# wizardyesterday/RtlSdrDiags

Hardware: AMD Instinct MI355X
Metric: IQ MSamples/s through WBFM chain at 1/2/4/8 GPUs; % HBM roofline (higher is better)
Workload: dtype int8/int16 Q15 + f32; 1 GPU; BASELINE configs[1]: WBFM, 1 channel, 2^28-sample synthetic IQ; channels_per_gpu=1, log2_samples_per_channel=28, kernels=streaming pipelines

## Files before the change

rtlsdrdiags_amd/csrc/iqd_engine.cpp:

```cpp
#include "iqdemod.h"

#include <hip/hip_runtime.h>
#include <math.h>
#include <stdarg.h>
#include <stdio.h>
#include <string.h>

#include <algorithm>
#include <mutex>
#include <string>
#include <vector>

#include "iqd_host.h"
#include "iqd_plan.h"
#include "iqd_kernels.h"
#include "iqd_stream.h"
#include "iqd_stream_mixed.h"
#include "iqd_taps.h"
#include "iqd_wbfm.h"
#include "iqd_chains.h"
#include "iqd_chan.h"

using namespace iqd;

// ... 61 lines not shown
    uint32_t *d_tracker = nullptr;
    AgcConfig *d_agc_cfg = nullptr;
    AgcState *d_agc = nullptr;
    GainEpoch *d_epochs = nullptr;
    std::vector<float> k_applied;
    std::vector<uint32_t> wbfm_epoch_left;
    std::vector<uint32_t> wbfm_epoch_seq;
    uint32_t accept_seq = 0;
    uint32_t *h_epoch_report = nullptr;
    bool epoch_report_pending = false;
    uint32_t epoch_report_seq = 0;
    std::vector<uint32_t> epoch_report_channels;
    uint32_t wbfm_epochs_live = 0;
    std::vector<int32_t> rot_applied;
    bool rot_changed = false;
    ScanConfig *d_scan_cfg = nullptr;
    ScanState *d_scan = nullptr;
    float *d_atan = nullptr, *d_fmlut = nullptr;
    float *d_half_lut = nullptr;
    uint32_t *d_amat[3] = {nullptr, nullptr, nullptr};
    uint32_t *d_amat4 = nullptr;
    D4Args d4_args{};
    std::vector<float> fm_kmax;
    bool stream_ok = false;
    std::vector<uint32_t> mode_gen, rot_gen;
    std::vector<float> wbfm_kmax;
    StreamArgs stream_args{};
    uint64_t stream_handoffs = 0;
    uint32_t *d_counters = nullptr;
    unsigned long long *d_stamps = nullptr;
    uint32_t *h_counters = nullptr;

    DevBuf stream_hist;
    DevBuf lists[FAM_COUNT + 1], mag_sums, blk_lists, vlen, records, base8k, base8k2, gain_trace, freq_trace, dc_records, dc_records2, repair_flags;
    size_t mag_sums_zero = 0;
    hipStream_t pre_stream = nullptr;
    hipEvent_t ev_pre_done[2] = {nullptr, nullptr}, ev_chain_done[2] = {nullptr, nullptr}, ev_main_decisions = nullptr;
    DevBuf g_sums[2], g_blk[2], g_vlen[2];
    int gate_set = 0;
    bool chain_pending[2] = {false, false};
    bool decisions_on_main = false;
    bool in_host_path = false;
    DevBuf st_iq, st_pcm, st_count, st_mag, st_allowed;
    DevBuf sl_iq[2], sl_pcm[2], sl_count[2], sl_mag[2], sl_allowed[2];
    hipStream_t copy_stream = nullptr;
    hipStream_t fam_stream[3] = {};
    hipEvent_t fam_fork = nullptr, fam_join[3] = {};
    hipEvent_t ev_in[2] = {nullptr, nullptr}, ev_free[2] = {nullptr, nullptr};
    uint32_t *h_slice_counts = nullptr;
    uint32_t *d_closed = nullptr, *h_closed = nullptr;
    size_t h_slice_counts_cap = 0;
    uint8_t *h_small = nullptr;
    size_t h_small_cap = 0;

    bool profiling = false;
    std::vector<std::pair<hipEvent_t, hipEvent_t>> ev_free_pairs, ev_pending;
    iqd_stats stats{};
    std::string last_error;

    int fail(int code, const char *fmt, ...)
    {
        char buf[512];
        va_list ap;
        va_start(ap, fmt);
        vsnprintf(buf, sizeof(buf), fmt, ap);
        va_end(ap);
        last_error = buf;
// ... 229 lines not shown
        ok = ok && hipMemcpyAsync(e->d_atan, atan_lut.data(), atan_lut.size() * sizeof(float),
                                  hipMemcpyHostToDevice, e->stream) == hipSuccess;
        ok = ok && hipMemcpyAsync(e->d_fmlut, fm_lut.data(), fm_lut.size() * sizeof(float),
                                  hipMemcpyHostToDevice, e->stream) == hipSuccess;
        ok = ok && hipMemcpyAsync(e->d_half_lut, half_lut.data(), half_lut.size() * sizeof(float),
                                  hipMemcpyHostToDevice, e->stream) == hipSuccess;
        for (int r = 0; r < 3; r++)
            ok = ok && hipMemcpyAsync(e->d_amat[r], amat[r].data(), amat[r].size() * sizeof(uint32_t),
                                      hipMemcpyHostToDevice, e->stream) == hipSuccess;
        ok = ok && hipMemcpyAsync(e->d_amat4, amat4.data(), amat4.size() * sizeof(uint32_t), hipMemcpyHostToDevice,
                                  e->stream) == hipSuccess;
        ok = ok && upload_consts(e->consts, e->stream) == hipSuccess;
        ok = ok && hipStreamSynchronize(e->stream) == hipSuccess;
    }
    if (!ok) {
        iqd_destroy(e);
        return IQD_ENOMEM;
    }
    *out = e;
    return IQD_OK;
}

void iqd_destroy(iqd_t *e)
{
    if (!e) return;
    (void)hipSetDevice(e->device);
    if (e->stream) (void)hipStreamSynchronize(e->stream);
    void *ptrs[] = {e->d_params, e->d_tails, e->d_wcarry, e->d_dc, e->d_tracker, e->d_agc_cfg, e->d_agc, e->d_epochs, e->d_scan_cfg, e->d_scan,
                    e->d_atan, e->d_fmlut, e->d_counters, e->d_stamps, e->d_half_lut, e->d_amat[0], e->d_amat[1], e->d_amat[2], e->d_amat4};
    for (void *p : ptrs)
        if (p) (void)hipFree(p);
    if (e->h_counters) (void)hipHostFree(e->h_counters);
    for (auto &b : e->lists) b.release();
    DevBuf *bufs[] = {&e->stream_hist, &e->mag_sums, &e->blk_lists, &e->vlen, &e->records, &e->base8k, &e->base8k2, &e->gain_trace, &e->freq_trace, &e->dc_records, &e->dc_records2, &e->repair_flags,
                      &e->st_iq, &e->st_pcm, &e->st_count, &e->st_mag, &e->st_allowed};
    for (DevBuf *b : bufs) b->release();
    for (int b = 0; b < 2; b++) {
        e->sl_iq[b].release(); e->sl_pcm[b].release(); e->sl_count[b].release();
        e->sl_mag[b].release(); e->sl_allowed[b].release();
        if (e->ev_in[b]) (void)hipEventDestroy(e->ev_in[b]);
        if (e->ev_free[b]) (void)hipEventDestroy(e->ev_free[b]);
    }
    if (e->pre_stream) {
        (void)hipStreamSynchronize(e->pre_stream);
        (void)hipStreamDestroy(e->pre_stream);
        for (int k = 0; k < 2; k++) {
            (void)hipEventDestroy(e->ev_pre_done[k]);
            (void)hipEventDestroy(e->ev_chain_done[k]);
            e->g_sums[k].release(); e->g_blk[k].release(); e->g_vlen[k].release();
        }
        (void)hipEventDestroy(e->ev_main_decisions);
    }
    if (e->h_slice_counts) (void)hipHostFree(e->h_slice_counts);
    if (e->h_small) (void)hipHostFree(e->h_small);
    if (e->h_epoch_report) (void)hipHostFree(e->h_epoch_report);
    if (e->d_closed) (void)hipFree(e->d_closed);
    if (e->h_closed) (void)hipHostFree(e->h_closed);
    if (e->copy_stream) (void)hipStreamDestroy(e->copy_stream);
    for (int f = 0; f < 3; f++) {
        if (e->fam_stream[f]) (void)hipStreamDestroy(e->fam_stream[f]);
        if (e->fam_join[f]) (void)hipEventDestroy(e->fam_join[f]);
    }
    if (e->fam_fork) (void)hipEventDestroy(e->fam_fork);
    for (auto *v : {&e->ev_free_pairs, &e->ev_pending})
        for (auto &pr : *v) { (void)hipEventDestroy(pr.first); (void)hipEventDestroy(pr.second); }
    if (e->stream) (void)hipStreamDestroy(e->stream);
    delete e;
// ... 934 lines not shown
    }
    if (f == FAM_WBFM) {
        HIP_TRY(e, e->records.ensure((size_t)n_list * a.tiles_per_ch * sizeof(WbfmRecord)));
        a.records = e->records.as<WbfmRecord>();
        if (e->repair_flags.cap < n_list * sizeof(uint32_t)) {
            HIP_TRY(e, e->repair_flags.ensure(n_list * sizeof(uint32_t)));
            HIP_COPY(e, hipMemsetAsync(e->repair_flags.p, 0, e->repair_flags.cap, s));
        }
        a.repair_flags = e->repair_flags.as<uint32_t>();
        if (streams) {
            const int stream_rot = e->plan_shape.fam[FAM_WBFM].rot_first;
            StreamArgs sa = e->stream_args;
            sa.amat = e->d_amat[stream_rot + 1];
            sa.half_lut = e->d_half_lut;
            sa.n_segments = n_list * a.tiles_per_ch;
            sa.grouped = fp.grouped ? 1u : 0u;
            for (int r = 0; r < 3; r++) {
                sa.group_start[r] = fp.grouped ? fp.group_start[r] : 0u;
                sa.group_li0[r] = fp.grouped ? fp.group_li0[r] : 0u;
                sa.group_nseg[r] = fp.grouped ? fp.group_nseg[r] : 0u;
                sa.amat3[r] = e->d_amat[2 - r];
            }
            sa.group_start[3] = fp.grouped ? fp.group_start[3] : 0u;
            sa.rounds = fp.rounds;
            sa.rings = fp.rings;
            HIP_TRY(e, e->stream_hist.ensure((size_t)sa.n_segments * sizeof(StHist)));
            sa.hist = e->stream_hist.as<StHist>();
            a.verify_at_end = x.gated ? 2u : 1u;
            if (fused) {
                x.mix.a[f] = a;
                x.mix.sa = sa;
                x.mix.wbfm_rot = stream_rot;
            } else {
                HIP_LAUNCH(e, launch_wbfm_stream(a, sa, stream_rot, x.fused_mag, fp.epochs, fp.grid, s));
                HIP_LAUNCH(e, launch_wbfm_stream_fixup(a, sa, s));
            }
            if (!x.gated) e->stream_handoffs += (uint64_t)n_list * ((x.vlen + a.tile_len - 1) / a.tile_len - 1);
            e->stats.stream_launches++;
        } else {
            HIP_LAUNCH(e, launch_wbfm(a, x.gated, x.fused_mag, n_list * a.tiles_per_ch, s));
        }
    } else {
        D4Args d4 = e->d4_args;
        if (streams) {
            for (int r = 0; r < 3; r++) {
                d4.group_start[r] = fp.group_start[r];
                d4.group_li0[r] = fp.group_li0[r];
                d4.group_nseg[r] = fp.group_nseg[r];
            }
            d4.group_start[3] = fp.group_start[3];
            d4.amat = e->d_amat4 + (size_t)(f == FAM_FM ? 0 : 3) * 4 * 64 * 4;
            d4.fm_lut = e->d_fmlut;
            d4.halo = (int32_t)fp.halo;
            d4.lead_shift = fp.lead_shift;
            d4.rounds = fp.rounds;
            d4.rings = fp.rings;
        }
        if (f != FAM_FM) {
            int rc = attach_dc_buffers(e, x, f, a, s);
            if (rc != IQD_OK) return rc;
            if (streams) {
                a.base_stride_ch = x.base.pcm_stride;
                a.base_stride_t = 1;
                static const bool no_det16 = getenv("IQD_NO_DET16") != nullptr;
                a.det16 = a.dc_tiles < 2 && !no_det16 ? 1u : 0u;
            }
        }
        if (streams) {
// ... 431 lines not shown
```

rtlsdrdiags_amd/csrc/iqd_kernels.hip:

```cpp
#include <hip/hip_runtime.h>

#include "iqd_kernels.h"
#include "iqd_chains.h"
#include "iqd_wbfm.h"
#include "iqd_stream_fix.h"

namespace iqd {

__constant__ Consts g_consts;

hipError_t upload_consts(const Consts &c, hipStream_t s)
{
    return hipMemcpyToSymbolAsync(HIP_SYMBOL(g_consts), &c, sizeof(Consts), 0, hipMemcpyHostToDevice, s);
}

hipError_t consts_address(const Consts **p)
{
    void *a = nullptr;
    const hipError_t e = hipGetSymbolAddress(&a, HIP_SYMBOL(g_consts));
    *p = (const Consts *)a;
    return e;
}

struct DeviceExec {
// ... 477 lines not shown
{
    if (blockIdx.x < a.n_list) tail_update_body(a, family, blockIdx.x);
    else squelch_block_body(q, always_open, (blockIdx.x - a.n_list) * 256u + threadIdx.x);
}

__global__ __launch_bounds__(256) void tail_dc_squelch_kernel(const ChainLaunch a, int family, const SquelchLaunch q, int always_open)
{
    __shared__ DcLds lds;
    if (blockIdx.x < a.n_list) {
        if (threadIdx.x >= 64) return;
        dc_channel_wave(a, family, blockIdx.x, lds);
    } else if (blockIdx.x < 2 * a.n_list) {
        tail_update_body(a, family, blockIdx.x - a.n_list);
    } else {
        squelch_block_body(q, always_open, (blockIdx.x - 2 * a.n_list) * 256u + threadIdx.x);
    }
}

__global__ __launch_bounds__(WB_THREADS, IQD_WBFM_MIN_WAVES) void wbfm_repair_squelch_kernel(const ChainLaunch a, const SquelchLaunch q, int always_open)
{
    __shared__ WbfmLds lds;
    if (blockIdx.x < a.n_list) wbfm_repair_body<false>(a, lds, blockIdx.x);
    else squelch_block_body(q, always_open, (blockIdx.x - a.n_list) * 256u + threadIdx.x);
}

struct MixedTailRoles { uint32_t end[6]; };
__global__ __launch_bounds__(256) void mixed_tail_kernel(const ChainLaunch a_wbfm, const StreamArgs sa, const ChainLaunch a_am,
                                                         const ChainLaunch a_fm, const ChainLaunch a_ssb, const MixedTailRoles roles)
{
    __shared__ union Lds { DcLds dc; FixLds fix; __device__ Lds() {} } u;
    DcLds &lds = u.dc;
    const uint32_t b = blockIdx.x;
    if (b < roles.end[0]) {
        wbfm_stream_fixup_body(a_wbfm, sa, b, u.fix);
    } else if (b < roles.end[2]) {
        if (threadIdx.x >= 64) return;
        const int family = b < roles.end[1] ? FAM_AM : FAM_SSB;
        const ChainLaunch &a = family == FAM_AM ? a_am : a_ssb;
        const uint32_t li = b - (family == FAM_AM ? roles.end[0] : roles.end[1]);
        dc_channel_wave(a, family, li, lds);
    } else if (b < roles.end[3]) {
        tail_update_body(a_am, FAM_AM, b - roles.end[2]);
    } else if (b < roles.end[4]) {
        tail_update_body(a_fm, FAM_FM, b - roles.end[3]);
    } else if (b < roles.end[5]) {
        tail_update_body(a_ssb, FAM_SSB, b - roles.end[4]);
    }
}

__global__ void squelch_track_kernel(const SquelchLaunch q, int always_open)
{
    const uint32_t ch = blockIdx.x * blockDim.x + threadIdx.x;
    if (ch >= q.n_ch) return;
    const uint32_t ech = q.first_ch + ch;
    const AgcConfig cfg = q.agc_cfg[ech];
    if (always_open && !cfg.enabled) return;
    const ChanParams &p = q.params[ech];
    AgcState st = q.agc[ech];
    uint32_t gain = st.rx_gain;
    uint32_t tracking = q.tracker[ech];
    uint32_t open = 0;
    const ScanConfig sc = q.scan_cfg[ech];
    ScanState ss = q.scan[ech];
    for (uint32_t b = 0; b < q.n_blocks; b++) {
        const size_t idx = (size_t)ch * q.n_blocks + b;
        const uint32_t avg = q.mag_sums[idx] / q.block_samples;
        if (!always_open) {
// ... 534 lines not shown
```

rtlsdrdiags_amd/csrc/iqd_stream.h:

```cpp
#pragma once
#include <stdint.h>

#include "iqd_device.h"

namespace iqd {

constexpr int ST_WAVES = 15;
constexpr int ST_THREADS = 64 * ST_WAVES;
constexpr int ST_RINGS = 3;
constexpr int ST_P_PER_RING = 4;
constexpr int ST_SEGS = 64 * ST_RINGS;
constexpr int ST_HALO = FORCED_BACK;
#ifndef IQD_ST_AHEAD
#define IQD_ST_AHEAD 2
#endif
constexpr int ST_AHEAD = IQD_ST_AHEAD;
constexpr int ST_MIN_TILE = 768;
constexpr int ST_FIX_PCM = 21;
constexpr int ST_ROW_FLOATS = 260;
#ifndef IQD_ST_FAKE_SHIFT
#define IQD_ST_FAKE_SHIFT 0
#endif
constexpr int ST_LDS_ROW_FLOATS = IQD_ST_FAKE_SHIFT ? (256 >> IQD_ST_FAKE_SHIFT) + 4 : ST_ROW_FLOATS;
constexpr int ST_TABLE_BYTES = 129 * ST_LDS_ROW_FLOATS * 4;
constexpr int ST_SLOT_BYTES = 64 * 16 * 4;
#ifndef IQD_ST_DEPTH
#define IQD_ST_DEPTH 1
#endif
constexpr int ST_DEPTH = IQD_ST_DEPTH;
constexpr int ST_RING_SLOTS = 2 * ST_DEPTH;
constexpr int ST_SYNC_WORDS = 24;
constexpr int ST_LDS_BYTES = ST_TABLE_BYTES + ST_RINGS * ST_RING_SLOTS * ST_SLOT_BYTES + ST_SYNC_WORDS * 4;
static_assert(ST_LDS_BYTES <= 160 * 1024, "table + rings must fit the CU's LDS");
static_assert(ST_HALO % 128 == 0 && ST_HALO + 32 <= TAIL, "the lead-in is whole 128-sample units inside the kept tail");

struct StHist {
    uint32_t w_first[2];
    uint32_t y1_first[6];
    uint32_t y2_first[24];
    uint32_t y1_last[4];
    uint32_t w_last[2];
    uint32_t pad[6];
    uint32_t y2_last[20];
};
static_assert(sizeof(StHist) == 256, "one boundary record per segment, 256 bytes");

struct StreamArgs {
    StHist *hist;
    const uint32_t *amat;
    const float *half_lut;
    uint32_t n_segments;
    uint32_t rounds;
    uint32_t rings;
    uint32_t grouped;
    uint32_t group_start[4];
    uint32_t group_li0[3];
    uint32_t group_nseg[3];
    const uint32_t *amat3[3];
    uint32_t d1p[4];
    uint32_t d1p2[4];
    uint32_t p12p[6];
    uint32_t a40p[20];
    float b0, a1;
};

enum { D4_AM = 0, D4_SSB = 1, D4_FM = 2 };
constexpr int D4_HALO_AM = fir_halo(FAM_AM), D4_HALO_SSB = fir_halo(FAM_SSB), D4_HALO_FM = fir_halo(FAM_FM);
constexpr int D4_HALO_SHORT = 128;
constexpr int d4_full_halo(int family) { return family == FAM_FM ? D4_HALO_FM : family == FAM_AM ? D4_HALO_AM : D4_HALO_SSB; }
constexpr int d4_lead_shift(int family) { return d4_full_halo(family) - D4_HALO_SHORT; }
constexpr int D4_REPLAY_AM = 4, D4_REPLAY_SSB = 36, D4_REPLAY_FM = 20;
constexpr int D4_REPLAY_PAIRS_AMSSB = 4;
constexpr int D4_RAILS_FROM_PIECE = 8;
constexpr int d4_replay_outputs(int family) { return family == FAM_FM ? D4_REPLAY_FM : family == FAM_AM ? D4_REPLAY_AM : D4_REPLAY_SSB; }
struct D4Geom { int64_t v0; uint32_t skip, cold; };
#if defined(__HIPCC__)
__host__ __device__
#endif
inline D4Geom d4_geom(uint32_t sid, uint32_t tile, uint32_t tile_len, uint32_t shift)
{
    D4Geom g;
    if (!shift) { g.v0 = (int64_t)tile * tile_len; g.skip = 0; g.cold = 1; return g; }
    g.cold = tile == 0 || (sid & 63u) == 0 ? 1u : 0u;
    const uint32_t c = 1u + (sid >> 6) - ((sid - tile) >> 6);
    g.v0 = (int64_t)tile * tile_len - (int64_t)shift * c;
    g.skip = g.cold ? shift : 0u;
    return g;
}
constexpr uint32_t d4_max_cold(uint32_t n_tiles) { return 1u + (n_tiles + 62u) / 64u; }
struct D4Args {
    const uint32_t *amat;
    const float *fm_lut;
    uint32_t group_start[4];
    uint32_t group_li0[3];
    uint32_t group_nseg[3];
    uint32_t rounds;
// ... 16 lines not shown
```

rtlsdrdiags_amd/csrc/iqd_stream.hip:

```cpp
#include <hip/hip_runtime.h>

#include "iqd_kernels.h"
#include "iqd_stream.h"
#include "iqd_wbfm.h"
#include "iqd_mfma.h"
#include "iqd_stream_fix.h"
#include "iqd_taps.h"

namespace iqd {

#ifdef IQD_ST_WT_STORES
__device__ __forceinline__ void st_store16(void *p, v4u v)
{
    asm volatile("global_store_dwordx4 %0, %1, off sc1\n\ts_nop 1" :: "v"(p), "v"(v) : "memory");
}
#define ST_STORE16(P, A, B, C, D) st_store16((void *)(P), v4u{A, B, C, D})
#elif defined(IQD_ST_NT_STORES)
#define ST_STORE16(P, A, B, C, D) __builtin_nontemporal_store(v4u{A, B, C, D}, (v4u *)(P))
#else
#define ST_STORE16(P, A, B, C, D) (*(u32x4 *)(P) = u32x4{A, B, C, D})
#endif


typedef __attribute__((address_space(3))) const uint32_t lds_cu32;
// ... 670 lines not shown
__device__ __forceinline__ void wbfm_stream_body(const ChainLaunch &a, const StreamArgs &sa, uint8_t *st_lds)
{
    if ((uint32_t)(uintptr_t)(__attribute__((address_space(3))) uint8_t *)st_lds != 0u) __builtin_trap();
    uint32_t *sync = (uint32_t *)(st_lds + ST_TABLE_BYTES + ST_RINGS * ST_RING_SLOTS * ST_SLOT_BYTES);
    const int tid = (int)threadIdx.x;
    {
        constexpr int N16 = ST_TABLE_BYTES / 16, TRIPS = (N16 + ST_THREADS - 1) / ST_THREADS;
        uint4 t[TRIPS];
#pragma unroll
        for (int k = 0; k < TRIPS; k++) {
            const int i = tid + k * ST_THREADS;
            t[k] = ((const uint4 *)sa.half_lut)[i < N16 ? i : N16 - 1];
        }
#pragma unroll
        for (int k = 0; k < TRIPS; k++) {
            const int i = tid + k * ST_THREADS;
            if (i < N16) ((uint4 *)st_lds)[i] = t[k];
        }
    }
    if (tid < ST_SYNC_WORDS) sync[tid] = 0;
    __syncthreads();
    const int wave = __builtin_amdgcn_readfirstlane(tid >> 6), lane = tid & 63;
    uint32_t pc = 0;
    if (wave < ST_RINGS) st_iir_wave(a, sa, st_lds, sync, wave, lane, ROT != 2 && !GATED && !EPOCHS ? IQD_ST_COLD_HALO : ST_HALO);
    else if (ROT != 2) st_p_wave<ROT, MAG, EPOCHS, GATED>(a, sa, st_lds, sync, wave - ST_RINGS, lane, pc);
    else {
        st_p_wave<1, MAG, EPOCHS, GATED, true>(a, sa, st_lds, sync, wave - ST_RINGS, lane, pc);
        st_p_wave<0, MAG, EPOCHS, GATED, true>(a, sa, st_lds, sync, wave - ST_RINGS, lane, pc);
        st_p_wave<-1, MAG, EPOCHS, GATED, true>(a, sa, st_lds, sync, wave - ST_RINGS, lane, pc);
    }
}

#ifndef IQD_STREAM_BODIES_ONLY
template <int ROT, bool MAG, bool EPOCHS, bool GATED>
__global__ __launch_bounds__(ST_THREADS, 4) void wbfm_stream_kernel(const ChainLaunch a, const StreamArgs sa)
{
    extern __shared__ __attribute__((aligned(16))) uint8_t st_lds[];
    wbfm_stream_body<ROT, MAG, EPOCHS, GATED>(a, sa, st_lds);
}
#endif

#ifndef IQD_STREAM_BODIES_ONLY
__global__ __launch_bounds__(FIX_THREADS) void wbfm_stream_fixup_kernel(const ChainLaunch a, const StreamArgs sa)
{
    __shared__ FixLds fl;
    wbfm_stream_fixup_body(a, sa, blockIdx.x, fl);
}

hipError_t launch_wbfm_stream_fixup(const ChainLaunch &a, const StreamArgs &sa, hipStream_t s)
{
    hipLaunchKernelGGL(wbfm_stream_fixup_kernel, dim3((sa.n_segments + FIX_SEGS - 1) / FIX_SEGS), dim3(FIX_THREADS), 0, s, a, sa);
    return hipGetLastError();
}

typedef void (*StKernel)(const ChainLaunch, const StreamArgs);
#define ST_K(R) {{wbfm_stream_kernel<R, false, false, false>, wbfm_stream_kernel<R, false, true, false>}, \
                 {wbfm_stream_kernel<R, true, false, false>, wbfm_stream_kernel<R, true, true, false>},   \
                 {wbfm_stream_kernel<R, false, false, true>, wbfm_stream_kernel<R, false, true, true>}}
static const StKernel st_kernels[4][3][2] = {ST_K(-1), ST_K(0), ST_K(1), ST_K(2)};
#undef ST_K

hipError_t init_wbfm_stream_kernels()
{
    for (int r = 0; r < 4; r++)
        for (int g = 0; g < 6; g++) {
            const hipError_t e = hipFuncSetAttribute((const void *)st_kernels[r][g >> 1][g & 1], hipFuncAttributeMaxDynamicSharedMemorySize, ST_LDS_BYTES);
            if (e != hipSuccess) return e;
        }
    return hipSuccess;
}

hipError_t launch_wbfm_stream(const ChainLaunch &a, const StreamArgs &sa, int rotation, bool mag, bool epochs, uint32_t grid, hipStream_t s)
{
    const int variant = a.vlen_gated ? 2 : (mag ? 1 : 0);
    hipLaunchKernelGGL(st_kernels[sa.grouped ? 3 : rotation < 0 ? 0 : rotation > 0 ? 2 : 1][variant][epochs ? 1 : 0], dim3(grid), dim3(ST_THREADS), ST_LDS_BYTES, s, a, sa);
    return hipGetLastError();
}

#endif

}
```

rtlsdrdiags_amd/csrc/iqd_stream_fix.h:

```cpp
#pragma once
#include <hip/hip_runtime.h>

#include "iqd_kernels.h"
#include "iqd_stream.h"
#include "iqd_stream_mixed.h"
#include "iqd_wbfm.h"
#include "iqd_mfma.h"

namespace iqd {

struct StSeg {
    uint32_t valid, li, tile, ch, ech;
    int32_t v0, tlen;
    int32_t vlen;
};

__device__ __forceinline__ StSeg st_segment(const ChainLaunch &a, uint32_t sid, uint32_t n_segments)
{
    StSeg s;
    s.valid = sid < n_segments ? 1u : 0u;
    const uint32_t id = s.valid ? sid : 0u;
    s.li = id / a.tiles_per_ch;
    s.tile = id - s.li * a.tiles_per_ch;
    s.ch = a.ch_list[s.li];
    s.ech = a.first_ch + s.ch;
    const uint32_t vlen = a.vlen_gated ? a.vlen_gated[s.ch] : a.vlen;
    s.vlen = (int32_t)vlen;
    const int64_t v0 = (int64_t)s.tile * a.tile_len;
    if (v0 >= (int64_t)vlen) { s.valid = 0; s.v0 = 0; s.tlen = 0; return s; }
    s.v0 = (int32_t)v0;
    const int64_t rest = (int64_t)vlen - v0;
    s.tlen = (int32_t)(rest < (int64_t)a.tile_len ? rest : (int64_t)a.tile_len);
    if (!s.valid) s.tlen = 0;
    return s;
}

#ifndef IQD_ST_NO_GROUPS
#define IQD_ST_NO_GROUPS 0
#endif
__device__ __forceinline__ StSeg st_segment_of(const ChainLaunch &a, const StreamArgs &sa, uint32_t sid, int &rot)
{
    if (IQD_ST_NO_GROUPS || !sa.grouped) { rot = 0; return st_segment(a, sid, sa.n_segments); }
    const uint32_t r = (sid >= sa.group_start[1] ? 1u : 0u) + (sid >= sa.group_start[2] ? 1u : 0u);
    rot = 1 - (int)r;
    const uint32_t local = sid - sa.group_start[r];
    const bool there = sid < sa.group_start[3] && local < sa.group_nseg[r];
    return st_segment(a, there ? sa.group_li0[r] * a.tiles_per_ch + local : sa.n_segments, sa.n_segments);
}
__device__ __forceinline__ bool st_cold_and_full(const StSeg &s, uint32_t tile_len)
{
    if (!s.valid) return true;
    const bool not_last = s.vlen - s.v0 > s.tlen;
    const bool keeps_restart = not_last && s.vlen - FORCED_BACK >= s.v0 && s.vlen - FORCED_BACK < s.v0 + s.tlen;
    return s.tile != 0 && s.tlen == (int32_t)tile_len && !keeps_restart;
}
__device__ __forceinline__ uint32_t st_id_count(const StreamArgs &sa) { return !IQD_ST_NO_GROUPS && sa.grouped ? sa.group_start[3] : sa.n_segments; }

#ifndef IQD_FIX_LANES
#define IQD_FIX_LANES 16
#endif
constexpr int FIX_LANES = IQD_FIX_LANES;
constexpr int FIX_SEGS = 256 / FIX_LANES;
constexpr int FIX_THREADS = FIX_LANES * FIX_SEGS;
static_assert(FIX_LANES == 16 || FIX_LANES == 32, "threads per boundary");
struct FixLds {
    uint32_t rec[(FIX_SEGS + 1) * 64];
    uint32_t y2x[FIX_SEGS][41];
};
__device__ __forceinline__ void wbfm_stream_fixup_body(const ChainLaunch &a, const StreamArgs &sa, const uint32_t block, FixLds &fl)
{
    uint32_t (&rec)[(FIX_SEGS + 1) * 64] = fl.rec;
    uint32_t (&y2x)[FIX_SEGS][41] = fl.y2x;
    const uint32_t sid0 = block * FIX_SEGS;
    const int tid = (int)threadIdx.x, sl = tid / FIX_LANES, i = tid % FIX_LANES;
    const uint32_t sid = sid0 + (uint32_t)sl;
    const StSeg sg = st_segment(a, sid < sa.n_segments ? sid : 0u, sa.n_segments);
    const bool live = sid < sa.n_segments && sg.valid && sg.tile != 0;
    float y_in = 0.f, y_end = 0.f;
    if (live && i == FIX_LANES - 1) {
        const WbfmRecord *r = a.records + (size_t)sg.li * a.tiles_per_ch;
        y_in = r[sg.tile].y_in;
        y_end = r[sg.tile - 1].y_end;
    }
    {
        const uint32_t *src = (const uint32_t *)sa.hist + ((size_t)sid0 - (sid0 ? 1 : 0)) * 64;
        const uint32_t n_avail = (sa.n_segments - sid0 < (uint32_t)FIX_SEGS ? sa.n_segments - sid0 : (uint32_t)FIX_SEGS) + (sid0 ? 1u : 0u);
        for (uint32_t k = (uint32_t)tid; k < n_avail * 64; k += FIX_THREADS) rec[k + (sid0 ? 0 : 64)] = src[k];
    }
    __syncthreads();
    const StHist &prev = *(const StHist *)&rec[sl * 64], &own = *(const StHist *)&rec[(sl + 1) * 64];
    if (live && i < 3) {
        int acc = 1 << 14;
        acc = dot2(prev.w_last[0], sa.d1p[0], acc);
        acc = dot2(prev.w_last[1], sa.d1p[1], acc);
        acc = dot2(own.w_first[0], sa.d1p[2], acc);
        acc = dot2(own.w_first[1], sa.d1p[3], acc);
        uint32_t y1[10];
#pragma unroll
        for (int k = 0; k < 4; k++) y1[k] = prev.y1_last[k];
#pragma unroll
        for (int k = 0; k < 6; k++) y1[4 + k] = own.y1_first[k];
        y1[4] = (y1[4] & 0xffff0000u) | ((uint32_t)(acc >> 15) & 0xffffu);
        int s2 = 1 << 14;
#pragma unroll
        for (int q = 0; q < 6; q++) {
            const uint32_t d = i == 0 ? y1[5 - q] : (i == 1 ? y1[7 - q] : y1[9 - q]);
            s2 = dot2(d, sa.p12p[q], s2);
        }
        ((int16_t *)&y2x[sl][20])[i] = (int16_t)(s2 >> 15);
    } else if (live) {
        for (int p = i - 3; p < 41; p += FIX_LANES - 3) {
            if (p == 20) continue;
            if (p == 21) ((int16_t *)&y2x[sl][21])[1] = (int16_t)(own.y2_first[1] >> 16);
            else y2x[sl][p] = p < 20 ? prev.y2_last[p] : own.y2_first[p - 20];
        }
    }
    if (live && i == FIX_LANES - 1 && f2u(y_in) != f2u(y_end)) {
        if (!iir_states_agree(y_in, y_end, a.params[sg.ech].wbfm_k >= 1.0f)) {
            atomicAdd(&a.counters[CNT_TILE_MISMATCH], 1u);
            atomicAdd(&a.counters[CNT_STREAM_MISMATCH], 1u);
            a.repair_flags[sg.li] = 1;
        }
    }
    __syncthreads();
    if (!live) return;
    for (int j = i; j < ST_FIX_PCM && j < sg.tlen / 32; j += FIX_LANES) {
        int s3 = 1 << 14;
#pragma unroll
        for (int q = 0; q < 20; q++) {
            const uint32_t pair = y2x[sl][20 + j - q];
            s3 = clamp_q30(dot2(pair, sa.a40p[q] & 0xffff0000u, s3));
            s3 = clamp_q30(dot2(pair, sa.a40p[q] & 0x0000ffffu, s3));
        }
        a.pcm[(size_t)sg.ch * a.pcm_stride + (sg.v0 >> 5) + j] = (int16_t)(s3 >> 15);
    }
}

}
```

rtlsdrdiags_amd/csrc/iqd_taps.h:

```cpp
#pragma once

namespace iqd {
namespace taps {

constexpr float WBFM_PRE[16] = {
    -0.0157211f, -0.0325959f, 0.0092996f, 0.0621217f, -0.0148595f, -0.0989456f, 0.1182989f, 0.4862333f,
    0.4862333f, 0.1182989f, -0.0989456f, -0.0148595f, 0.0621217f, 0.0092996f, -0.0325959f, -0.0157211f};

constexpr float WBFM_D1[8] = {0.0243699f, 0.0769537f, 0.1463572f, 0.1967096f,
                              0.1967096f, 0.1463572f, 0.0769537f, 0.0243699f};

constexpr float POST12[12] = {0.0022977f, 0.0237042f, 0.0605386f, 0.1127073f, 0.1645167f, 0.1971107f,
                              0.1971107f, 0.1645167f, 0.1127073f, 0.0605386f, 0.0237042f, 0.0022977f};

constexpr float AUDIO40[40] = {
    0.0015969f, -0.0111080f, -0.0270501f, -0.0265610f, -0.0023190f, 0.0180618f, 0.0065495f, -0.0183409f,
    -0.0133345f, 0.0184489f, 0.0230891f, -0.0161248f, -0.0363745f, 0.0091343f, 0.0550219f, 0.0070312f,
    -0.0862280f, -0.0497761f, 0.1793543f, 0.4145808f, 0.4145808f, 0.1793543f, -0.0497761f, -0.0862280f,
    0.0070312f, 0.0550219f, 0.0091343f, -0.0363745f, -0.0161248f, 0.0230891f, 0.0184489f, -0.0133345f,
    -0.0183409f, 0.0065495f, 0.0180618f, -0.0023190f, -0.0265610f, -0.0270501f, -0.0111080f, 0.0015969f};

constexpr float FM_TUNER[32] = {
    0.0041331f, 0.0054174f, 0.0076016f, 0.0115481f, 0.0151685f, 0.0203192f, 0.0251608f, 0.0311322f,
    0.0366372f, 0.0427168f, 0.0480527f, 0.0533425f, 0.0575831f, 0.0611914f, 0.0635413f, 0.0648239f,
    0.0648239f, 0.0635413f, 0.0611914f, 0.0575831f, 0.0533425f, 0.0480527f, 0.0427168f, 0.0366372f,
    0.0311322f, 0.0251608f, 0.0203192f, 0.0151685f, 0.0115481f, 0.0076016f, 0.0054174f, 0.0041331f};

constexpr float AM_S1[8] = {0.0242683f, 0.0766338f, 0.1457589f, 0.1959036f,
                            0.1959036f, 0.1457589f, 0.0766338f, 0.0242683f};
constexpr float AM_S2[12] = {0.0057496f, 0.0263853f, 0.0605301f, 0.1074406f, 0.1523486f, 0.1804951f,
                             0.1804951f, 0.1523486f, 0.1074406f, 0.0605301f, 0.0263853f, 0.0057496f};
constexpr float AM_S3[16] = {0.0116487f, 0.0152694f, -0.0109804f, -0.0611915f, -0.0736143f, 0.0187617f,
                             0.1988190f, 0.3481364f, 0.3481364f, 0.1988190f, 0.0187617f, -0.0736143f,
                             -0.0611915f, -0.0109804f, 0.0152694f, 0.0116487f};

constexpr float SSB_DELAY[16] = {0, 0, 0, 0, 0, 0, 0, 0, 0, 0, 0, 0, 0, 0, 0, 1};
constexpr float SSB_HILBERT[31] = {
    -0.0033953f, 0, -0.0058652f, 0, -0.0134385f, 0, -0.0281423f, 0, -0.0534836f, 0, -0.0980394f, 0,
    -0.1935638f, 0, -0.6302204f, 0, 0.6302204f, 0, 0.1935638f, 0, 0.0980394f, 0, 0.0534836f, 0,
    0.0281423f, 0, 0.0134385f, 0, 0.0058652f, 0, 0.0033953f};

constexpr float DEEMPH_B0 = 0.0253863f;
constexpr float DEEMPH_A1 = -0.9492274f;
constexpr float DCBLOCK_A1 = -0.95f;

constexpr int q15(float h)
{
    const float s = h * 32768.0f;
    return (int)(s + (s >= 0.f ? 0.5f : -0.5f));
}
constexpr unsigned pair16(int lo, int hi) { return ((unsigned)lo & 0xffffu) | ((unsigned)hi << 16); }
struct StreamTaps {
    unsigned d1p2[4], p12p[6], a40p[20];
    constexpr StreamTaps() : d1p2{}, p12p{}, a40p{}
    {
        for (int q = 0; q < 4; q++) d1p2[q] = pair16(2 * q15(WBFM_D1[7 - 2 * q]), 2 * q15(WBFM_D1[6 - 2 * q]));
        for (int q = 0; q < 6; q++) p12p[q] = pair16(q15(POST12[2 * q + 1]), q15(POST12[2 * q]));
        for (int q = 0; q < 20; q++) a40p[q] = pair16(q15(AUDIO40[2 * q + 1]), q15(AUDIO40[2 * q]));
    }
};
constexpr StreamTaps STREAM_TAPS{};

}
}
```

rtlsdrdiags_amd/csrc/iqd_wbfm.h:

```cpp
#pragma once
#include "iqd_device.h"
#include "iqd_prims.h"

namespace iqd {

#ifndef IQD_WB_THREADS
#define IQD_WB_THREADS 256
#endif
constexpr int WB_THREADS = IQD_WB_THREADS;
constexpr int WB_BIAS = 2 * (16384 + (128 << 15));
constexpr int TGRAN = TSTRIDE / 4;

IQD_DEV int t_slot(int seg, int gi) { return seg * TGRAN + (gi ^ ((gi >> 3) & 3)); }

struct WbfmLds {
    u32x4 t4[WBFM_NSEG * TGRAN];
    alignas(16) uint32_t w[WBFM_NSEG * WSTRIDE];
    alignas(16) uint32_t y1[(8 + WBFM_CHUNK / 4) / 2];
    alignas(16) uint32_t y2[(40 + WBFM_CHUNK / 16) / 2];
    uint32_t whist[4];
    float z[WBFM_NSEG + 4];
    float g[WBFM_NSEG];
    float e[WBFM_NSEG];
    float y_carry, u_carry;
// ... 599 lines not shown
        lds.y2_peak_hist = lds.y2_peak > keep ? lds.y2_peak : keep;
        lds.y2_peak = 0;
    }
}

struct WbfmStart {
    float y, u;
    int32_t back;
    int32_t cold;
};

struct WbfmRecord {
    float y_in;
    float y_out, u_out;
    int32_t back_out;
    float y_end, u_end;
    uint32_t pad[2];
};
constexpr uint32_t WBFM_REC_STREAMED = 0x53545245u;

struct StRecPlan { int32_t rec_pos, back_out, park_pos; uint32_t keeps_restart; };
IQD_DEV StRecPlan st_rec_plan(uint32_t valid, uint32_t tile, int32_t v0, int32_t tlen, int32_t vlen, int32_t carried_back)
{
    StRecPlan r;
    const int32_t halo = tile == 0 ? carried_back : FORCED_BACK;
    r.rec_pos = tlen - FORCED_BACK;
    if (r.rec_pos < -halo) r.rec_pos = -halo;
    r.back_out = tlen - r.rec_pos;
    const bool not_last = vlen - v0 > tlen;
    r.keeps_restart = valid && not_last && vlen - FORCED_BACK >= v0 && vlen - FORCED_BACK < v0 + tlen ? 1u : 0u;
    r.park_pos = r.keeps_restart ? vlen - FORCED_BACK - v0 : r.rec_pos;
    return r;
}

IQD_DEV WbfmCarry wbfm_pick_carry(const WbfmRecord &last, const WbfmRecord &before, uint32_t ntiles, uint32_t vlen, uint32_t tile_len,
                                  uint32_t verify_at_end)
{
    WbfmCarry cy;
    cy.y = last.y_out; cy.u = last.u_out; cy.back = last.back_out;
    if (verify_at_end && ntiles >= 2 && last.pad[0] == WBFM_REC_STREAMED && vlen - (ntiles - 1) * tile_len < (uint32_t)FORCED_BACK) {
        cy.y = u2f(before.pad[0]); cy.u = u2f(before.pad[1]); cy.back = FORCED_BACK;
    }
    cy.y_end = last.y_end; cy.u_end = last.u_end;
    cy.pad[0] = cy.pad[1] = cy.pad[2] = 0;
    return cy;
}

IQD_DEV float epoch_gain(const GainEpochList *ep, float k_now, int v)
{
    float k = k_now;
    if (ep)
        for (int i = 0; i < EPOCHS; i++) {
            if (ep->since[i] >= (uint32_t)TAIL || v >= -(int)ep->since[i]) break;
            k = ep->k_before[i];
        }
    return k;
}
IQD_DEV float epoch_gain_search(const GainEpochList *ep, float k_now, int v)
{
    static_assert((EPOCHS & (EPOCHS - 1)) == 0, "a power of two");
    const uint32_t want = (uint32_t)(v < 0 ? -v : 0);
    int m = 0;
#pragma unroll
    for (int step = EPOCHS / 2; step >= 1; step >>= 1)
        m += ep->since[m + step - 1] < want ? step : 0;
    m += m == EPOCHS - 1 && ep->since[EPOCHS - 1] < want ? 1 : 0;
// ... 400 lines not shown
```

Measured before the change: 830,900 MSamples/s.

## Fold WBFM stream boundary fixup into the stream kernel epilogue with tickets

Runs the boundary fixup pass at the end of each streaming WBFM workgroup instead of in a separate fixup kernel launch. Neighbouring workgroups coordinate through atomic ticket counters, so whichever finishes second handles the shared edge segment, with acquire fences for visibility. Filter taps in the epilogue become compile-time literals. This removes a kernel launch and a dependent pass over the history data, but adds atomics, fences, a tickets buffer that is never re-zeroed and uses ticket parity, and extra tail work in the stream kernel.

```diff
diff --git a/rtlsdrdiags_amd/csrc/iqd_engine.cpp b/rtlsdrdiags_amd/csrc/iqd_engine.cpp
--- a/rtlsdrdiags_amd/csrc/iqd_engine.cpp
+++ b/rtlsdrdiags_amd/csrc/iqd_engine.cpp
@@ -117,7 +117,7 @@
     uint32_t *h_counters = nullptr;
 
     DevBuf stream_hist;
-    DevBuf lists[FAM_COUNT + 1], mag_sums, blk_lists, vlen, records, base8k, base8k2, gain_trace, freq_trace, dc_records, dc_records2, repair_flags;
+    DevBuf lists[FAM_COUNT + 1], mag_sums, blk_lists, vlen, records, base8k, base8k2, gain_trace, freq_trace, dc_records, dc_records2, repair_flags, fix_tickets;
     size_t mag_sums_zero = 0;
     hipStream_t pre_stream = nullptr;
     hipEvent_t ev_pre_done[2] = {nullptr, nullptr}, ev_chain_done[2] = {nullptr, nullptr}, ev_main_decisions = nullptr;
@@ -413,7 +413,7 @@
         if (p) (void)hipFree(p);
     if (e->h_counters) (void)hipHostFree(e->h_counters);
     for (auto &b : e->lists) b.release();
-    DevBuf *bufs[] = {&e->stream_hist, &e->mag_sums, &e->blk_lists, &e->vlen, &e->records, &e->base8k, &e->base8k2, &e->gain_trace, &e->freq_trace, &e->dc_records, &e->dc_records2, &e->repair_flags,
+    DevBuf *bufs[] = {&e->stream_hist, &e->mag_sums, &e->blk_lists, &e->vlen, &e->records, &e->base8k, &e->base8k2, &e->gain_trace, &e->freq_trace, &e->dc_records, &e->dc_records2, &e->repair_flags, &e->fix_tickets,
                       &e->st_iq, &e->st_pcm, &e->st_count, &e->st_mag, &e->st_allowed};
     for (DevBuf *b : bufs) b->release();
     for (int b = 0; b < 2; b++) {
@@ -1414,8 +1414,18 @@
                 x.mix.sa = sa;
                 x.mix.wbfm_rot = stream_rot;
             } else {
+                static const bool epilogue_fix = !(getenv("IQD_ST_EPILOGUE_FIX") && atoi(getenv("IQD_ST_EPILOGUE_FIX")) == 0);
+                sa.fix_in_kernel = epilogue_fix && !fp.grouped && fp.rounds <= ST_FIX_MAX_ROUNDS ? 1u : 0u;
+                if (sa.fix_in_kernel) {
+                    const size_t ticket_bytes = (size_t)st_fix_ticket_words(sa.n_segments) * sizeof(uint32_t);
+                    if (e->fix_tickets.cap < ticket_bytes) {
+                        HIP_TRY(e, e->fix_tickets.ensure(ticket_bytes));
+                        HIP_COPY(e, hipMemsetAsync(e->fix_tickets.p, 0, e->fix_tickets.cap, s));
+                    }
+                    sa.fix_tickets = e->fix_tickets.as<uint32_t>();
+                }
                 HIP_LAUNCH(e, launch_wbfm_stream(a, sa, stream_rot, x.fused_mag, fp.epochs, fp.grid, s));
-                HIP_LAUNCH(e, launch_wbfm_stream_fixup(a, sa, s));
+                if (!sa.fix_in_kernel) HIP_LAUNCH(e, launch_wbfm_stream_fixup(a, sa, s));
             }
             if (!x.gated) e->stream_handoffs += (uint64_t)n_list * ((x.vlen + a.tile_len - 1) / a.tile_len - 1);
             e->stats.stream_launches++;
diff --git a/rtlsdrdiags_amd/csrc/iqd_kernels.hip b/rtlsdrdiags_amd/csrc/iqd_kernels.hip
--- a/rtlsdrdiags_amd/csrc/iqd_kernels.hip
+++ b/rtlsdrdiags_amd/csrc/iqd_kernels.hip
@@ -533,7 +533,7 @@
     DcLds &lds = u.dc;
     const uint32_t b = blockIdx.x;
     if (b < roles.end[0]) {
-        wbfm_stream_fixup_body(a_wbfm, sa, b, u.fix);
+        wbfm_stream_fixup_body<FIX_SEGS, false>(a_wbfm, sa, b * FIX_SEGS, 0u, sa.n_segments, u.fix);
     } else if (b < roles.end[2]) {
         if (threadIdx.x >= 64) return;
         const int family = b < roles.end[1] ? FAM_AM : FAM_SSB;
diff --git a/rtlsdrdiags_amd/csrc/iqd_stream.h b/rtlsdrdiags_amd/csrc/iqd_stream.h
--- a/rtlsdrdiags_amd/csrc/iqd_stream.h
+++ b/rtlsdrdiags_amd/csrc/iqd_stream.h
@@ -16,6 +16,7 @@
 #endif
 constexpr int ST_AHEAD = IQD_ST_AHEAD;
 constexpr int ST_MIN_TILE = 768;
+constexpr uint32_t ST_FIX_MAX_ROUNDS = ST_THREADS / 2;
 constexpr int ST_FIX_PCM = 21;
 constexpr int ST_ROW_FLOATS = 260;
 #ifndef IQD_ST_FAKE_SHIFT
@@ -62,6 +63,9 @@
     uint32_t p12p[6];
     uint32_t a40p[20];
     float b0, a1;
+    uint32_t *fix_tickets;
+    uint32_t fix_in_kernel;
+    uint32_t fix_pad;
 };
 
 enum { D4_AM = 0, D4_SSB = 1, D4_FM = 2 };
diff --git a/rtlsdrdiags_amd/csrc/iqd_stream.hip b/rtlsdrdiags_amd/csrc/iqd_stream.hip
--- a/rtlsdrdiags_amd/csrc/iqd_stream.hip
+++ b/rtlsdrdiags_amd/csrc/iqd_stream.hip
@@ -726,11 +726,58 @@
 }
 
 #ifndef IQD_STREAM_BODIES_ONLY
+#ifndef IQD_ST_EPI_FENCE_ALL
+#define IQD_ST_EPI_FENCE_ALL 0
+#endif
+constexpr int EPI_SEGS = ST_THREADS / FIX_LANES;
+static_assert(EPI_SEGS <= 64, "at least two passes, whatever the rings");
+static_assert(sizeof(FixLdsT<EPI_SEGS>) + 2 * ST_FIX_MAX_ROUNDS * 4 <= (size_t)ST_LDS_BYTES, "the epilogue's scratch fits the kernel's LDS");
+__device__ __forceinline__ void wbfm_stream_epilogue(const ChainLaunch &a, const StreamArgs &sa, uint8_t *st_lds)
+{
+    if (IQD_ST_EPI_FENCE_ALL) __builtin_amdgcn_fence(__ATOMIC_RELEASE, "agent");
+    __syncthreads();
+    FixLdsT<EPI_SEGS> &fl = *(FixLdsT<EPI_SEGS> *)st_lds;
+    uint32_t *second = (uint32_t *)(st_lds + sizeof(FixLdsT<EPI_SEGS>));
+    const uint32_t tid = threadIdx.x;
+    const uint32_t n_pass = st_fix_passes(sa.rings, (uint32_t)EPI_SEGS);
+    uint32_t ticket = 0;
+    if (tid < 2u * sa.rounds) {
+        const StFixRound fr = st_fix_round(chain_wg(a), chain_wgs(a), tid >> 1, sa.rings, sa.n_segments);
+        const uint32_t sid = tid & 1u ? fr.end : fr.first;
+        const StSeg succ = st_segment(a, sid, sa.n_segments);
+        if (fr.runs && st_fix_live(succ.valid, succ.tile))
+            ticket = __hip_atomic_fetch_add(sa.fix_tickets + (tid & 1u ? fr.back_word : fr.front_word), 1u, __ATOMIC_RELEASE, __HIP_MEMORY_SCOPE_AGENT);
+    }
+    for (uint32_t round = 0; round < sa.rounds; round++) {
+        const StFixRound fr = st_fix_round(chain_wg(a), chain_wgs(a), round, sa.rings, sa.n_segments);
+        if (!fr.runs) break;
+        for (uint32_t p = 1; p + 1 < n_pass; p++) {
+            wbfm_stream_fixup_body<EPI_SEGS, true>(a, sa, fr.first + p * (uint32_t)EPI_SEGS, fr.first + 1u, fr.end, fl);
+            __syncthreads();
+        }
+    }
+    if (tid < 2u * sa.rounds) second[tid] = ticket & 1u;
+    __syncthreads();
+    for (uint32_t round = 0; round < sa.rounds; round++) {
+        const StFixRound fr = st_fix_round(chain_wg(a), chain_wgs(a), round, sa.rings, sa.n_segments);
+        if (!fr.runs) break;
+        const uint32_t front = second[2u * round], back = second[2u * round + 1u];
+        if (IQD_ST_EPI_FENCE_ALL || (front | back))
+            __builtin_amdgcn_fence(__ATOMIC_ACQUIRE, "agent");
+        const uint32_t lo = fr.first + 1u - front, hi = fr.end + back;
+        wbfm_stream_fixup_body<EPI_SEGS, true>(a, sa, fr.first, lo, hi, fl);
+        __syncthreads();
+        wbfm_stream_fixup_body<EPI_SEGS, true>(a, sa, fr.first + (n_pass - 1u) * (uint32_t)EPI_SEGS, lo, hi, fl);
+        __syncthreads();
+    }
+}
+
 template <int ROT, bool MAG, bool EPOCHS, bool GATED>
 __global__ __launch_bounds__(ST_THREADS, 4) void wbfm_stream_kernel(const ChainLaunch a, const StreamArgs sa)
 {
     extern __shared__ __attribute__((aligned(16))) uint8_t st_lds[];
     wbfm_stream_body<ROT, MAG, EPOCHS, GATED>(a, sa, st_lds);
+    if (ROT != 2 && sa.fix_in_kernel) wbfm_stream_epilogue(a, sa, st_lds);
 }
 #endif
 
@@ -738,7 +785,7 @@
 __global__ __launch_bounds__(FIX_THREADS) void wbfm_stream_fixup_kernel(const ChainLaunch a, const StreamArgs sa)
 {
     __shared__ FixLds fl;
-    wbfm_stream_fixup_body(a, sa, blockIdx.x, fl);
+    wbfm_stream_fixup_body<FIX_SEGS, false>(a, sa, blockIdx.x * FIX_SEGS, 0u, sa.n_segments, fl);
 }
 
 hipError_t launch_wbfm_stream_fixup(const ChainLaunch &a, const StreamArgs &sa, hipStream_t s)
@@ -767,6 +814,7 @@
 hipError_t launch_wbfm_stream(const ChainLaunch &a, const StreamArgs &sa, int rotation, bool mag, bool epochs, uint32_t grid, hipStream_t s)
 {
     const int variant = a.vlen_gated ? 2 : (mag ? 1 : 0);
+    if (sa.fix_in_kernel && (sa.grouped || sa.rounds > ST_FIX_MAX_ROUNDS || !sa.fix_tickets)) return hipErrorInvalidValue;
     hipLaunchKernelGGL(st_kernels[sa.grouped ? 3 : rotation < 0 ? 0 : rotation > 0 ? 2 : 1][variant][epochs ? 1 : 0], dim3(grid), dim3(ST_THREADS), ST_LDS_BYTES, s, a, sa);
     return hipGetLastError();
 }
diff --git a/rtlsdrdiags_amd/csrc/iqd_stream_fix.h b/rtlsdrdiags_amd/csrc/iqd_stream_fix.h
--- a/rtlsdrdiags_amd/csrc/iqd_stream_fix.h
+++ b/rtlsdrdiags_amd/csrc/iqd_stream_fix.h
@@ -6,6 +6,7 @@
 #include "iqd_stream_mixed.h"
 #include "iqd_wbfm.h"
 #include "iqd_mfma.h"
+#include "iqd_taps.h"
 
 namespace iqd {
 
@@ -63,19 +64,25 @@
 constexpr int FIX_SEGS = 256 / FIX_LANES;
 constexpr int FIX_THREADS = FIX_LANES * FIX_SEGS;
 static_assert(FIX_LANES == 16 || FIX_LANES == 32, "threads per boundary");
-struct FixLds {
-    uint32_t rec[(FIX_SEGS + 1) * 64];
-    uint32_t y2x[FIX_SEGS][41];
+template <int SEGS>
+struct FixLdsT {
+    uint32_t rec[(SEGS + 1) * 64];
+    uint32_t y2x[SEGS][41];
 };
-__device__ __forceinline__ void wbfm_stream_fixup_body(const ChainLaunch &a, const StreamArgs &sa, const uint32_t block, FixLds &fl)
+typedef FixLdsT<FIX_SEGS> FixLds;
+template <int SEGS, bool LIT>
+__device__ __forceinline__ void wbfm_stream_fixup_body(const ChainLaunch &a, const StreamArgs &sa, const uint32_t sid0, const uint32_t lo,
+                                                       const uint32_t hi, FixLdsT<SEGS> &fl)
 {
-    uint32_t (&rec)[(FIX_SEGS + 1) * 64] = fl.rec;
-    uint32_t (&y2x)[FIX_SEGS][41] = fl.y2x;
-    const uint32_t sid0 = block * FIX_SEGS;
+#define FIX_TAP(WHICH, Q) (LIT ? (uint32_t)taps::STREAM_TAPS.WHICH[Q] : sa.WHICH[Q])
+    constexpr uint32_t THREADS = (uint32_t)(SEGS * FIX_LANES);
+    uint32_t (&rec)[(SEGS + 1) * 64] = fl.rec;
+    uint32_t (&y2x)[SEGS][41] = fl.y2x;
     const int tid = (int)threadIdx.x, sl = tid / FIX_LANES, i = tid % FIX_LANES;
     const uint32_t sid = sid0 + (uint32_t)sl;
-    const StSeg sg = st_segment(a, sid < sa.n_segments ? sid : 0u, sa.n_segments);
-    const bool live = sid < sa.n_segments && sg.valid && sg.tile != 0;
+    const bool mine = sid >= lo && sid < hi && sid < sa.n_segments;
+    const StSeg sg = st_segment(a, mine ? sid : 0u, sa.n_segments);
+    const bool live = mine && sg.valid && sg.tile != 0;
     float y_in = 0.f, y_end = 0.f;
     if (live && i == FIX_LANES - 1) {
         const WbfmRecord *r = a.records + (size_t)sg.li * a.tiles_per_ch;
@@ -83,18 +90,22 @@
         y_end = r[sg.tile - 1].y_end;
     }
     {
-        const uint32_t *src = (const uint32_t *)sa.hist + ((size_t)sid0 - (sid0 ? 1 : 0)) * 64;
-        const uint32_t n_avail = (sa.n_segments - sid0 < (uint32_t)FIX_SEGS ? sa.n_segments - sid0 : (uint32_t)FIX_SEGS) + (sid0 ? 1u : 0u);
-        for (uint32_t k = (uint32_t)tid; k < n_avail * 64; k += FIX_THREADS) rec[k + (sid0 ? 0 : 64)] = src[k];
+        const uint32_t from = sid0 > lo ? sid0 : lo;
+        uint32_t to = sid0 + (uint32_t)SEGS < hi ? sid0 + (uint32_t)SEGS : hi;
+        to = to < sa.n_segments ? to : sa.n_segments;
+        const uint32_t r0 = from ? from - 1u : 0u;
+        const uint32_t *src = (const uint32_t *)sa.hist + (size_t)r0 * 64;
+        const uint32_t n_words = to > r0 ? (to - r0) * 64u : 0u;
+        for (uint32_t k = (uint32_t)tid; k < n_words; k += THREADS) rec[k + (r0 + 1u - sid0) * 64u] = src[k];
     }
     __syncthreads();
     const StHist &prev = *(const StHist *)&rec[sl * 64], &own = *(const StHist *)&rec[(sl + 1) * 64];
     if (live && i < 3) {
         int acc = 1 << 14;
-        acc = dot2(prev.w_last[0], sa.d1p[0], acc);
-        acc = dot2(prev.w_last[1], sa.d1p[1], acc);
-        acc = dot2(own.w_first[0], sa.d1p[2], acc);
-        acc = dot2(own.w_first[1], sa.d1p[3], acc);
+        acc = dot2(prev.w_last[0], FIX_TAP(d1p, 0), acc);
+        acc = dot2(prev.w_last[1], FIX_TAP(d1p, 1), acc);
+        acc = dot2(own.w_first[0], FIX_TAP(d1p, 2), acc);
+        acc = dot2(own.w_first[1], FIX_TAP(d1p, 3), acc);
         uint32_t y1[10];
 #pragma unroll
         for (int k = 0; k < 4; k++) y1[k] = prev.y1_last[k];
@@ -105,7 +116,7 @@
 #pragma unroll
         for (int q = 0; q < 6; q++) {
             const uint32_t d = i == 0 ? y1[5 - q] : (i == 1 ? y1[7 - q] : y1[9 - q]);
-            s2 = dot2(d, sa.p12p[q], s2);
+            s2 = dot2(d, FIX_TAP(p12p, q), s2);
         }
         ((int16_t *)&y2x[sl][20])[i] = (int16_t)(s2 >> 15);
     } else if (live) {
@@ -129,11 +140,12 @@
 #pragma unroll
         for (int q = 0; q < 20; q++) {
             const uint32_t pair = y2x[sl][20 + j - q];
-            s3 = clamp_q30(dot2(pair, sa.a40p[q] & 0xffff0000u, s3));
-            s3 = clamp_q30(dot2(pair, sa.a40p[q] & 0x0000ffffu, s3));
+            s3 = clamp_q30(dot2(pair, FIX_TAP(a40p, q) & 0xffff0000u, s3));
+            s3 = clamp_q30(dot2(pair, FIX_TAP(a40p, q) & 0x0000ffffu, s3));
         }
         a.pcm[(size_t)sg.ch * a.pcm_stride + (sg.v0 >> 5) + j] = (int16_t)(s3 >> 15);
     }
+#undef FIX_TAP
 }
 
 }
diff --git a/rtlsdrdiags_amd/csrc/iqd_taps.h b/rtlsdrdiags_amd/csrc/iqd_taps.h
--- a/rtlsdrdiags_amd/csrc/iqd_taps.h
+++ b/rtlsdrdiags_amd/csrc/iqd_taps.h
@@ -52,8 +52,10 @@
 constexpr unsigned pair16(int lo, int hi) { return ((unsigned)lo & 0xffffu) | ((unsigned)hi << 16); }
 struct StreamTaps {
     unsigned d1p2[4], p12p[6], a40p[20];
-    constexpr StreamTaps() : d1p2{}, p12p{}, a40p{}
+    unsigned d1p[4];
+    constexpr StreamTaps() : d1p2{}, p12p{}, a40p{}, d1p{}
     {
+        for (int q = 0; q < 4; q++) d1p[q] = pair16(q15(WBFM_D1[7 - 2 * q]), q15(WBFM_D1[6 - 2 * q]));
         for (int q = 0; q < 4; q++) d1p2[q] = pair16(2 * q15(WBFM_D1[7 - 2 * q]), 2 * q15(WBFM_D1[6 - 2 * q]));
         for (int q = 0; q < 6; q++) p12p[q] = pair16(q15(POST12[2 * q + 1]), q15(POST12[2 * q]));
         for (int q = 0; q < 20; q++) a40p[q] = pair16(q15(AUDIO40[2 * q + 1]), q15(AUDIO40[2 * q]));
diff --git a/rtlsdrdiags_amd/csrc/iqd_wbfm.h b/rtlsdrdiags_amd/csrc/iqd_wbfm.h
--- a/rtlsdrdiags_amd/csrc/iqd_wbfm.h
+++ b/rtlsdrdiags_amd/csrc/iqd_wbfm.h
@@ -655,6 +655,21 @@
     r.park_pos = r.keeps_restart ? vlen - FORCED_BACK - v0 : r.rec_pos;
     return r;
 }
+
+struct StFixRound { uint32_t runs, first, end, front_word, back_word; };
+IQD_DEV StFixRound st_fix_round(uint32_t wg, uint32_t wgs, uint32_t round, uint32_t rings, uint32_t n_ids)
+{
+    StFixRound r;
+    r.first = (round * wgs + wg) * 64u * rings;
+    r.end = r.first + 64u * rings;
+    r.runs = r.first < n_ids ? 1u : 0u;
+    r.front_word = r.first >> 6;
+    r.back_word = r.end >> 6;
+    return r;
+}
+IQD_DEV bool st_fix_live(uint32_t valid, uint32_t tile) { return valid != 0 && tile != 0; }
+IQD_DEV uint32_t st_fix_passes(uint32_t rings, uint32_t per_pass) { return (64u * rings + 1u + per_pass - 1u) / per_pass; }
+constexpr uint32_t st_fix_ticket_words(uint32_t n_ids) { return (n_ids >> 6) + 2u; }
 
 IQD_DEV WbfmCarry wbfm_pick_carry(const WbfmRecord &last, const WbfmRecord &before, uint32_t ntiles, uint32_t vlen, uint32_t tile_len,
                                   uint32_t verify_at_end)
```

Result: slower. 766,000 MSamples/s (-7.8%).
